# stefantaubert/waveglow

Measured on AMD Instinct MI355X. Metric: audio samples/sec/GPU (22.05 kHz) WaveGlow-256 infer; real-time factor, higher is better.
Workload: dtype f16 MFMA operands, f32 accumulate/flow state, fp16 I/O; 1 GPU; configs[1]: 256ch WaveGlow.infer, batch=16/GPU mels 80x864, fp16 I/O, sigma=0.6; parallelism=utterance-sharded x1, no collective

## Files before the change

### waveglow_amd/csrc/api.cpp

```cpp
#include <cmath>
#include <cstdarg>
#include <cstring>

#include "wg_host.h"

using namespace wg;

namespace {
thread_local std::string g_err;
}

int wg::fail(int code, const char* fmt, ...) {
  char buf[512];
  va_list ap;
  va_start(ap, fmt);
  vsnprintf(buf, sizeof buf, fmt, ap);
  va_end(ap);
  g_err = buf;
  return code;
}

namespace {

bool invert(const std::vector<double>& A, int n, std::vector<double>& inv, double& logabsdet, int& sign) {
// ... 195 lines not shown
  if (c.n_flows < 1 || c.n_early_every < 1 || c.n_early_size < 0 || c.n_early_size % 2 != 0)
    return fail(WG_ERR_INVALID, "bad flow configuration");
  std::vector<int> ck = flow_channels(c);
  if (ck.back() < 2 || ck.back() % 2 != 0) return fail(WG_ERR_INVALID, "flow configuration leaves %d channels", ck.back());
  wg_handle* h = new wg_handle();
  h->cfg = c;
  h->device = device_id;
  {
    int ncu = 0;
    if (hipDeviceGetAttribute(&ncu, hipDeviceAttributeMultiprocessorCount, device_id) == hipSuccess && ncu > 0) h->n_cu = ncu;
  }
  h->NS = c.n_mel_channels * c.n_group;
  h->c_k = ck;
  if (const char* e = getenv("WG_FORCE_BN")) h->force_bn = atoi(e);
  if (const char* e = getenv("WG_NO_START_FOLD")) h->fold_start = !(*e == '1');
  h->expected.push_back("upsample.weight");
  h->expected.push_back("upsample.bias");
  for (int k = 0; k < c.n_flows; ++k) {
    const std::string ks = std::to_string(k);
    h->expected.push_back("convinv." + ks + ".conv.weight");
    const std::string p = "WN." + ks + ".";
    for (const char* n : {"start", "cond_layer", "end"}) {
      h->expected.push_back(p + n + ".weight");
      h->expected.push_back(p + n + ".bias");
    }
    for (int i = 0; i < c.n_layers; ++i) {
      const std::string is = std::to_string(i);
      h->expected.push_back(p + "in_layers." + is + ".weight");
      h->expected.push_back(p + "in_layers." + is + ".bias");
      h->expected.push_back(p + "res_skip_layers." + is + ".weight");
// ... 329 lines not shown
}

size_t wg_infer_workspace_bytes(const wg_handle* h, int32_t B, int32_t n_frames) {
  if (!h || B < 1 || n_frames < 1) return 0;
  const int L = n_frames * h->cfg.upsample_stride / h->cfg.n_group;
  RowGeom g = make_geom(h->cfg, B, L, n_frames);
  return carve(h, g, nullptr).bytes;
}

size_t wg_forward_workspace_bytes(const wg_handle* h, int32_t B, int32_t n_frames, int32_t audio_len) {
  if (!h || B < 1 || n_frames < 1 || audio_len < h->cfg.n_group || audio_len % h->cfg.n_group) return 0;
  RowGeom g = make_geom(h->cfg, B, audio_len / h->cfg.n_group, n_frames);
  return carve(h, g, nullptr).bytes;
}

static int run_wn(wg_handle* h, int k, const RowGeom& g, Workspace& w, _Float16*& cur, _Float16*& oth, hipStream_t s) {
  const wg_config& c = h->cfg;
  const int C = c.n_channels;
  int BN = wn_block_n(C);
  if (BN == 128) {
    const int64_t t128 = (int64_t)kPhases * (g.Rp / 128), ncu = h->n_cu > 0 ? h->n_cu : 1;
    const int64_t r128 = (t128 + ncu - 1) / ncu, r64 = (2 * t128 + ncu - 1) / ncu;
    if (t128 < 4 * ncu && 6 * r64 < 10 * r128) BN = 64;
  }
  if (BN == 128 && h->force_bn == 64) BN = 64;
  if (h->force_bn == 128 && wn_block_n(C) == 128) BN = 128;
  const FlowOffsets& fo = h->flows[k];
  for (int i = 0; i < c.n_layers; ++i) {
    const LayerOffsets& lo = fo.layers[i];
    WnLayerArgs a;
    a.x_in = cur;
// ... 14 lines not shown
    a.out = w.OUT;
    a.g = g;
    a.dil = 1 << i;
    a.n_cond_steps = c.n_mel_channels / 16;
    a.M = c.n_mel_channels;
    a.has_res = i < c.n_layers - 1;
    a.row0 = 0;
    a.tiles_per_phase = g.Rp / BN;
    a.sp = nullptr;
    a.save_t = a.save_s = a.save_a = nullptr;
    a.in0 = a.in1 = nullptr;
    a.out0 = nullptr;
    a.n_tiles = kPhases * a.tiles_per_phase;
    a.stamps = h->dbg_stamps;
    a.n_cu = h->n_cu;
    {
      Prof p(h, s, 2);
      HIP_TRY(launch_wn_layer(a, C, BN, s));
    }
    WG_DBG(s, "wn_layer");
    if (a.has_res) std::swap(cur, oth);
  }
  return WG_OK;
}

int wg_infer(wg_handle* h, const void* mel, const void* z_init, const void* const* z_early, int32_t n_z_early,
             float sigma, void* audio, int32_t B, int32_t n_frames, int32_t io_dtype, void* workspace,
             size_t workspace_bytes, void* stream) {
  return wg_infer_ragged(h, mel, nullptr, z_init, z_early, n_z_early, sigma, audio, B, n_frames, io_dtype, workspace,
                         workspace_bytes, stream);
// ... 57 lines not shown
    FlowArgs f = base_flow_args();
    f.first = 1;
    f.z_extra = z_init;
    f.c_next = h->c_k[k];
    f.h_next = f.c_next / 2;
    f.wstart = (const float*)(h->d_blob + h->flows[k].wstart);
    f.bstart = (const float*)(h->d_blob + h->flows[k].bstart);
    f.out_init = (const float*)(h->d_blob + h->flows[k].out_init);
    f.x = cur;
    f.a0p = w.A0;
    f.skip_x = h->fold_start && wn_res_a0(C);
    Prof p(h, s, 1);
    HIP_TRY(launch_flow(f, s));
  }
  WG_DBG(s, "flow");
  for (int k = c.n_flows - 1; k >= 0; --k) {
    int rc = run_wn(h, k, g, w, cur, oth, s);
    if (rc) return rc;
    FlowArgs f = base_flow_args();
    f.c_in = h->c_k[k];
    f.h_in = f.c_in / 2;
    f.winv = (const float*)(h->d_blob + h->flows[k].winv);
    if (is_early(c, k)) {
      f.z_extra = z_early[ze_idx++];
      f.n_extra = c.n_early_size;
      if (!f.z_extra) return fail(WG_ERR_INVALID, "null early-noise tensor");
    }
    f.c_next = f.c_in + f.n_extra;
    f.last = (k == 0);
    if (f.last) {
      if (f.c_next != c.n_group) return fail(WG_ERR_STATE, "flow bookkeeping error");
      f.audio_out = audio;
    } else {
      f.h_next = h->c_k[k - 1] / 2;
      if (h->c_k[k - 1] != f.c_next) return fail(WG_ERR_STATE, "flow bookkeeping error");
      f.wstart = (const float*)(h->d_blob + h->flows[k - 1].wstart);
      f.bstart = (const float*)(h->d_blob + h->flows[k - 1].bstart);
      f.out_init = (const float*)(h->d_blob + h->flows[k - 1].out_init);
      f.x = cur;
      f.a0p = w.A0;
      f.skip_x = h->fold_start && wn_res_a0(C);
    }
    Prof p(h, s, 1);
    HIP_TRY(launch_flow(f, s));
  }
  WG_DBG(s, "flow");
  return WG_OK;
}

int wg_forward(wg_handle* h, const void* mel, const void* audio, float* z, float* const* log_s, float* log_det_W,
               int32_t B, int32_t n_frames, int32_t audio_len, int32_t io_dtype, void* workspace,
               size_t workspace_bytes, void* stream) {
  if (!h) return fail(WG_ERR_INVALID, "null handle");
  if (!h->finalized) return fail(WG_ERR_STATE, "wg_finalize has not been called");
  if (!mel || !audio || !z || !log_s || !log_det_W || !workspace) return fail(WG_ERR_INVALID, "null buffer");
  if (io_dtype != WG_F32 && io_dtype != WG_F16) return fail(WG_ERR_INVALID, "bad io_dtype");
  const wg_config& c = h->cfg;
// ... 160 lines not shown
```

### waveglow_amd/csrc/kernels.hip

```cpp
#include "wg_common.h"

#include <cstdlib>
#include <type_traits>

namespace wg {

typedef _Float16 half8 __attribute__((ext_vector_type(8)));
typedef _Float16 half4 __attribute__((ext_vector_type(4)));
typedef float f32x16 __attribute__((ext_vector_type(16)));
typedef float f32x4 __attribute__((ext_vector_type(4)));

#define WG_GPTR(p) ((const __attribute__((address_space(1))) void*)(p))
#define WG_LPTR(p) ((__attribute__((address_space(3))) void*)(p))

__device__ __forceinline__ float load_io(const void* p, size_t i, int f16) {
  return f16 ? (float)((const _Float16*)p)[i] : ((const float*)p)[i];
}

__device__ __forceinline__ float gate_act(float u, float v) {
  const float e1 = __builtin_amdgcn_exp2f(__builtin_amdgcn_fmed3f(u, -60.0f, 60.0f));
  const float t = 1.0f + __builtin_amdgcn_exp2f(v);
  return (e1 - 1.0f) * __builtin_amdgcn_rcpf(fmaf(e1, t, t));
}

__device__ __forceinline__ void gate_act3(float u, float v, float& th, float& sg, float& ac) {
  const float e1 = __builtin_amdgcn_exp2f(__builtin_amdgcn_fmed3f(u, -60.0f, 60.0f));
  const float t = 1.0f + __builtin_amdgcn_exp2f(__builtin_amdgcn_fmed3f(v, -60.0f, 60.0f));
  const float r = __builtin_amdgcn_rcpf(fmaf(e1, t, t));
  ac = fmaf(e1, r, -r);
  sg = fmaf(e1, r, r);
  th = ac * t;
}

__device__ __forceinline__ void glds16(const void* sbase, unsigned voff, unsigned lds_addr) {
  unsigned keep;
  asm volatile("s_mov_b32 %0, m0\n\ts_mov_b32 m0, %3\n\ts_nop 2\n\tglobal_load_lds_dwordx4 %1, %2\n\ts_mov_b32 m0, %0"
               : "=&s"(keep) : "v"(voff), "s"(sbase), "s"(lds_addr) : "memory");
}
template <int OFF>
__device__ __forceinline__ void gload16(half8& dst, const void* sbase, unsigned voff) {
  asm volatile("s_nop 4\n\tglobal_load_dwordx4 %0, %1, %2 offset:%3" : "=v"(dst) : "v"(voff), "s"(sbase), "i"(OFF) : "memory");
}

#ifdef WG_STAMPS
#define WG_STAMP(i)                                                                              \
  do {                                                                                           \
    __builtin_amdgcn_sched_barrier(0);                                                           \
    unsigned long long _t;                                                                       \
    asm volatile("s_memtime %0\n\ts_waitcnt lgkmcnt(0)" : "=s"(_t)::"memory");                   \
    if (a.stamps && HAS_RES && tid == 0) a.stamps[(size_t)tile * 8 + (i)] = _t;                        \
    __builtin_amdgcn_sched_barrier(0);                                                           \
  } while (0)
#else
#define WG_STAMP(i) do {} while (0)
#endif

constexpr int kTilesPerWG = 2;


__device__ __forceinline__ void mfma16_acc(f32x4& c, const half8& a, const half8& b) {
  c = __builtin_amdgcn_mfma_f32_16x16x32_f16(a, b, c, 0, 0, 0);
}

template <int C> struct WnCfg {
  static constexpr int NW = (C >= 256) ? 8 : C / 32;
  static constexpr int BN = (C >= 512) ? 64 : 128;
};

template <int N> __device__ __forceinline__ void wait_vm() {
  asm volatile("s_waitcnt vmcnt(%0)" :: "i"(N) : "memory");
  __builtin_amdgcn_sched_barrier(0);
// ... 7 lines not shown
  constexpr int MT = PLAIN ? MB : 2 * MB;
  constexpr int NTHREADS = NW * 64;
  constexpr int NT = BN / 32;
  constexpr int CC = CX;
  constexpr int NKX = NTAPS * CC;
  constexpr int BT_BYTES = BN * 128;
  constexpr int ACT_ROW = 2 * C + 16;
  constexpr int K2 = C / 16;
  constexpr int NG = BN * 8 / NTHREADS;
  constexpr int NAH = MT * 2;
  constexpr bool DEFER = (MB == 1);
  static_assert(BN * 8 % NTHREADS == 0 && MB >= 1 && MB <= 2 && NKX >= 1 && (NTAPS == 1 || NTAPS == 3), "tile geometry");
  constexpr bool Q2L = !M16 && DEFER && !DEEP && (NG + NT - 1) / NT == 1 && NT >= NG + MT;
  static_assert(!M16 || (MODE == 0 && MB == 1 && DEFER && !DEEP && NT >= 2), "16x16x32 variant");
  constexpr bool A0G = MODE == 0 && CX == 1 && NTAPS == 1;
  static_assert(!DEEP || (MODE == 0 && DEFER && HAS_COND && MT <= NT && NG <= NT && ((NKX >= 4 && NKX % 2 == 0) || NKX == 1)), "deep prefetch variant");
  static_assert(MODE == 0 || (TPW == 1 && CX == ((MODE == 2 || MODE == 4) ? 2 : 1) * (C / 64)) || (MODE == 3 && CX == 1), "training variants");

  extern __shared__ __attribute__((aligned(16))) char smem[];
  char* const sB = smem;
  char* const sActs = MODE == 4 ? smem : smem + 2 * BT_BYTES;

  const int tid = threadIdx.x;
  const int wave = __builtin_amdgcn_readfirstlane(tid >> 6);
  int lane = tid & 63, ln = lane & 31, lh = lane >> 5;

  unsigned pvoff[NG];
  int pchunk[NG];
  int swB;
  int l15 = lane & 15, l4 = lane >> 4;
// ... 80 lines not shown
  auto column_of = [&](int rr, int p, int& b, int& t) -> bool {
    int rem = rr - tile_b0 * Fp;
    b = tile_b0;
    if (fp_ge_bn) {
      if (rem >= Fp) { rem -= Fp; ++b; }
    } else {
      const int qd = rem / Fp;
      b += qd;
      rem -= qd * Fp;
    }
    const int fq = rem - a.g.Gf;
    t = fq * 32 + p;
    if (!(b < a.g.B && fq >= 0 && fq < a.g.F && t < a.g.L)) return false;
    return a.g.frames == nullptr || t < 32 * a.g.frames[b];
  };

  int tile, tile_end;
  const int tile_step = gridDim.x >> 3;
  int run_start, run_quarter = 0;
  {
    const int bid = blockIdx.x, ntl = a.n_tiles;
    const int xcd = bid & 7, idx = bid >> 3;
    const int qq = ntl >> 3, r = ntl & 7;
    const int start = xcd < r ? xcd * (qq + 1) : r * (qq + 1) + (xcd - r) * qq;
    tile_end = start + (xcd < r ? qq + 1 : qq);
    tile = start + idx;
    run_start = start;
    if (((tile_end - start) & 3) == 0) run_quarter = (tile_end - start) >> 2;
  }
  auto tile_of = [&](int t) { return run_quarter ? run_start + ((t - run_start) & 3) * run_quarter + ((t - run_start) >> 2) : t; };

  half8 q[4][MT];
  int par = 0;
  if (tile < tile_end) {
    const int t0 = tile_of(tile), p0 = t0 / a.tiles_per_phase;
#pragma unroll
    for (int i = 0; i < NG; ++i) stage_B_piece(p0, t0 - p0 * a.tiles_per_phase, 0, 0, i);
  }
  float* const sBias = (float*)(sActs + BN * ACT_ROW);
  if constexpr (!PLAIN) {
    for (int i = tid; i < 2 * C; i += NTHREADS) sBias[i] = a.bias1[i];
    if constexpr (HAS_RES)
      for (int i = tid; i < C; i += NTHREADS) sBias[2 * C + i] = a.bias2[i];
    uint4* const sW = (uint4*)(sBias + 3 * C);
    for (int i = tid; i < (C / 32) * 64; i += NTHREADS) sW[i] = ((const uint4*)a.wEs)[i];
  }
  __syncthreads();

#pragma unroll
  for (int it = 0; it < TPW; ++it, tile += tile_step) {
    if (tile >= tile_end) break;
    if (it > 0) set_lane_ids();
    const int tile_m = tile_of(tile);
    const int p = tile_m / a.tiles_per_phase;
    const int jt = tile_m - p * a.tiles_per_phase;
    const int rr0 = a.row0 + jt * BN;
    tile_b0 = rr0 / Fp;
    const int r0 = kRowPad + p * Rp + rr0;
    const int next_tile = tile + tile_step;
    wA1c_p = (const char*)a.wA1c + (MODE != 0 ? (size_t)0 : (size_t)p * (2 * a.n_cond_steps) * NW * (NAH * 1024));
// ... 431 lines not shown
    const int l15 = laneo & 15, l4 = laneo >> 4;
    char* const acts_lane16 = sActs + l15 * ACT_ROW + (l4 & 1) * 32 + (l4 >> 1) * 8;
    auto write_acts16 = [&](int c, int blk_, int mh, const half8& o) {
      typedef _Float16 half4_t __attribute__((ext_vector_type(4)));
      const half4_t lo = {o[0], o[1], o[2], o[3]}, hi = {o[4], o[5], o[6], o[7]};
      char* ap = acts_lane16 + c * 32 * ACT_ROW + blk_ * 64 + mh * 16;
      *(half4_t*)(ap) = lo;
      *(half4_t*)(ap + 16 * ACT_ROW) = hi;
    };
    constexpr int NGRP = (BN / 16 + NW - 1) / NW;
    constexpr bool kWesEarly = (C / 32) * 4 <= 32;
    half8 wes[C / 32];
    float4 es_o[NGRP];
    float4* es_op[NGRP];
    bool es_valid[NGRP];
    auto es_prefetch_w = [&](int s_) { wes[s_] = ((const half8*)(sBias + 3 * C) + laneo)[s_ * 64]; };
    auto es_prefetch = [&]() {
#pragma unroll
      for (int gi = 0; gi < NGRP; ++gi) {
        const int grp = wave + gi * NW;
        es_valid[gi] = false;
        es_o[gi] = make_float4(0.f, 0.f, 0.f, 0.f);
        es_op[gi] = nullptr;
        if (grp < BN / 16) {
          int cb, ct;
          es_valid[gi] = column_of(rr0 + grp * 16 + l15, p, cb, ct) && laneo < 32;
          es_op[gi] = (float4*)(a.out + ((size_t)cb * a.g.L + ct) * 8 + 4 * l4);
          if (es_valid[gi]) es_o[gi] = *es_op[gi];
        }
      }
    };
    auto es_compute = [&]() {
#pragma unroll
      for (int s = 0; s < C / 32; ++s) es_prefetch_w(s);
#pragma unroll
      for (int gi = 0; gi < NGRP; ++gi) {
        const int grp = wave + gi * NW;
        if (grp < BN / 16) {
          const char* ep = sActs + (grp * 16 + l15) * ACT_ROW + l4 * 16;
          f32x4 d = {0.f, 0.f, 0.f, 0.f};
#pragma unroll
          for (int s = 0; s < C / 32; ++s) {
            const half8 bfe = *(const half8*)(ep + s * 64);
            d = __builtin_amdgcn_mfma_f32_16x16x32_f16(wes[s], bfe, d, 0, 0, 0);
          }
#pragma unroll
          for (int r = 0; r < 4; ++r) d[r] += __shfl_xor(d[r], 32);
          if (es_valid[gi]) {
            float4 o = es_o[gi];
            o.x += d[0]; o.y += d[1]; o.z += d[2]; o.w += d[3];
            *es_op[gi] = o;
          }
        }
      }
    };
    auto read_acts32 = [&](int nt, int k16) -> half8 {
      return *(const half8*)(acts_rd + nt * 32 * ACT_ROW + k16 * 32);
    };
    constexpr int PF = 8 / MB;
    half8 xres[RES_A0 ? 1 : MB][RES_A0 ? 1 : NT][2];
    half8 a0f[RES_A0 ? NT : 1], wst[RES_A0 ? MB : 1];
    half8 a2[MB][PF];
    const half8* const p2 = (const half8*)a.wA2 + (size_t)wave * MB * K2 * 64 + laneo;
    f32x16 acc2[MB][NT];
    if constexpr (PIPE) {
      constexpr int SL = 16;
      const int blk = wave;
// ... 260 lines not shown
#pragma unroll
        for (int mb = 0; mb < MB; ++mb) {
          const half8 af = a2[mb][k % PF];
          if (k + PF < K2) a2[mb][k % PF] = p2[((size_t)mb * K2 + k + PF) * 64];
#pragma unroll
          for (int nt = 0; nt < NT; ++nt)
            acc2[mb][nt] = __builtin_amdgcn_mfma_f32_32x32x16_f16(af, bq[k & 1][nt], acc2[mb][nt], 0, 0, 0);
        }
      }
    }

    if constexpr (!PIPE) {
      WG_STAMP(4);
      if constexpr (!kWesEarly) es_prefetch();
      es_compute();
    }

    if constexpr (!PIPE) WG_STAMP(5);
    if constexpr (HAS_RES && !PIPE) {
#pragma unroll
      for (int nt = 0; nt < NT; ++nt) {
        int cb, ct;
        if (column_of(rr0 + nt * 32 + lno, p, cb, ct)) {
#pragma unroll
          for (int mb = 0; mb < MB; ++mb) {
            const int blk = wave * MB + mb;
            half8 o0, o1;
#pragma unroll
            for (int r = 0; r < 8; ++r) {
              o0[r] = (_Float16)acc2[mb][nt][r];
// ... 8 lines not shown
      }
    }
    if constexpr (!PIPE) WG_STAMP(6);
    }
    __builtin_amdgcn_sched_barrier(0);
  }
}

template <int C, int BN, bool HAS_RES, int TPW, int CX, int MODE = 0, int NTAPS = 3, bool HAS_COND = true, bool DEEP = false>
static hipError_t launch_wn_tttt(const WnLayerArgs& a, hipStream_t s) {
  constexpr int NW = WnCfg<C>::NW;
  constexpr bool M16 = wn_frag16(C, BN) && MODE == 0 && !DEEP;
  if (M16 != (a.frag16 != 0)) return hipErrorInvalidValue;
  if (MODE == 0 && CX == 1 && NTAPS == 1 && wn_res_a0(C) && HAS_RES && !a.wStA) return hipErrorInvalidValue;
  constexpr int smem = MODE == 4 ? (BN * (2 * C + 16) > 2 * BN * 128 ? BN * (2 * C + 16) : 2 * BN * 128)
                                 : 2 * BN * 128 + (MODE >= 2 ? 0 : BN * (2 * C + 16) + 3 * C * 4 + (C / 32) * 1024);
  static bool attr_done_dev[64] = {};
  int cur_dev = 0;
  if (hipGetDevice(&cur_dev) != hipSuccess || cur_dev < 0 || cur_dev >= 64) cur_dev = 0;
  bool& attr_done = attr_done_dev[cur_dev];
  if (!attr_done) {
    hipError_t e = hipFuncSetAttribute((const void*)wn_layer_kernel<C, NW, BN, HAS_RES, TPW, CX, MODE, NTAPS, HAS_COND, DEEP, M16>,
                                       hipFuncAttributeMaxDynamicSharedMemorySize, smem);
    if (e != hipSuccess) return e;
    attr_done = true;
  }
  const int per_label = ((a.n_tiles + 7) / 8 + TPW - 1) / TPW;
  const int grid = 8 * per_label;
  hipLaunchKernelGGL((wn_layer_kernel<C, NW, BN, HAS_RES, TPW, CX, MODE, NTAPS, HAS_COND, DEEP, M16>), dim3(grid), dim3(NW * 64), smem, s, a);
  return hipGetLastError();
}
// ... 85 lines not shown
  if ((kind != 2 && kind != 3 && kind != 4) || !a.out0 || !a.x_tap || (kind == 3 && (!a.in0 || !a.in1))) return hipErrorInvalidValue;
  if ((kind == 2 || kind == 4) && (a.x_chunks_per_tap != 2 * (C / 64) || a.n_cond_steps != 0)) return hipErrorInvalidValue;
  if (kind == 4 && (!a.wat_prev || !a.gout || !a.t_prev || !a.s_prev || !a.dpre_prev)) return hipErrorInvalidValue;
  if (kind == 3 && !((a.x_chunks_per_tap == 1 && a.n_cond_steps == 0) || (a.x_chunks_per_tap == C / 64 && a.n_cond_steps == 1 && a.sp)))
    return hipErrorInvalidValue;
  switch (C) {
    case 64: return launch_wn_plain_t<64>(a, kind, bn, s);
    case 128: return launch_wn_plain_t<128>(a, kind, bn, s);
    case 256: return launch_wn_plain_t<256>(a, kind, bn, s);
    case 512: return launch_wn_plain_t<512>(a, kind, bn, s);
  }
  return hipErrorInvalidValue;
}

hipError_t launch_wn_layer(const WnLayerArgs& a, int C, int bn, hipStream_t s) {
  switch (C) {
    case 64: return launch_wn_t<64>(a, bn, s);
    case 128: return launch_wn_t<128>(a, bn, s);
    case 256: return launch_wn_t<256>(a, bn, s);
    case 512: return launch_wn_t<512>(a, bn, s);
  }
  return hipErrorInvalidValue;
}

__global__ void __launch_bounds__(256) mel_pack_kernel(const MelPackArgs a) {
  const int rows_per_utt = a.T + 6;
  const size_t n = (size_t)(3 + a.B * rows_per_utt) * a.M;
  for (size_t idx = (size_t)blockIdx.x * 256 + threadIdx.x; idx < n; idx += (size_t)gridDim.x * 256) {
    const int i = (int)(idx % a.M);
    const int row = (int)(idx / a.M) - 3;
// ... 142 lines not shown

template <int FL_ROWS>
__global__ void __launch_bounds__(FL_ROWS) flow_kernel(const FlowArgs a) {
  __shared__ float4 s_a0[FL_ROWS];
  const int L = a.g.L;
  const size_t nrows = (size_t)a.g.B * L;
  const size_t row0 = (size_t)blockIdx.x * FL_ROWS;
  const int tid = threadIdx.x;

  {
    const size_t row = row0 + tid;
    if (row < nrows) {
      const unsigned r32 = (unsigned)row;
      const int b = (int)(r32 / (unsigned)L), t = (int)(r32 - (unsigned)b * (unsigned)L);
      const bool pad_row = a.g.frames != nullptr && t >= 32 * a.g.frames[b];
      float zn[kMaxGroup];
#pragma unroll
      for (int c = 0; c < kMaxGroup; ++c) zn[c] = 0.0f;
      if (a.direction == 0) {
        if (a.first) {
#pragma unroll
          for (int c = 0; c < kMaxGroup; ++c)
            if (c < a.c_next)
              zn[c] = a.sigma * load_io(a.z_extra, ((size_t)b * a.c_next + c) * L + t, a.io_f16);
        } else {
          float z[kMaxGroup], o[kMaxGroup], v[kMaxGroup], y[kMaxGroup];
          const float4* zp = (const float4*)(a.Z + row * 8);
          const float4* op = (const float4*)(a.out + row * 8);
          float4 z0 = zp[0], z1 = zp[1], o0 = op[0], o1 = op[1];
          z[0] = z0.x; z[1] = z0.y; z[2] = z0.z; z[3] = z0.w; z[4] = z1.x; z[5] = z1.y; z[6] = z1.z; z[7] = z1.w;
          o[0] = o0.x; o[1] = o0.y; o[2] = o0.z; o[3] = o0.w; o[4] = o1.x; o[5] = o1.y; o[6] = o1.z; o[7] = o1.w;
          const int h = a.h_in, c = a.c_in;
#pragma unroll
          for (int j = 0; j < kMaxGroup; ++j) {
            float num = z[j], den = 1.0f;
#pragma unroll
            for (int q = 0; q < 4; ++q)
              if (j >= h && j - h == q) { num = z[j] - o[q]; den = expf(o[j]); }
            v[j] = (j < c) ? num / den : 0.0f;
          }
#pragma unroll
          for (int r = 0; r < kMaxGroup; ++r) {
            float s = 0.0f;
#pragma unroll
            for (int cc = 0; cc < kMaxGroup; ++cc)
              if (r < c && cc < c) s = fmaf(a.winv[r * c + cc], v[cc], s);
            y[r] = s;
          }
          const int ne = a.n_extra;
#pragma unroll
          for (int e = 0; e < kMaxGroup; ++e) {
            float val = 0.0f;
            if (e < ne) val = a.sigma * load_io(a.z_extra, ((size_t)b * ne + e) * L + t, a.io_f16);
#pragma unroll
            for (int r = 0; r < kMaxGroup; ++r)
              if (e >= ne && e - ne == r) val = y[r];
            zn[e] = val;
          }
        }
        if (a.last) {
          if (pad_row) {
#pragma unroll
            for (int c = 0; c < 8; ++c) zn[c] = 0.0f;
          }
          if (a.io_f16) {
            half8 o;
#pragma unroll
            for (int c = 0; c < 8; ++c) o[c] = (_Float16)zn[c];
            *(half8*)((_Float16*)a.audio_out + row * 8) = o;
          } else {
            float4* ap = (float4*)((float*)a.audio_out + row * 8);
            ap[0] = make_float4(zn[0], zn[1], zn[2], zn[3]);
            ap[1] = make_float4(zn[4], zn[5], zn[6], zn[7]);
          }
        }
      } else {
        float z[kMaxGroup];
        if (a.first) {
#pragma unroll
          for (int c = 0; c < 8; ++c)
            z[c] = load_io(a.audio_in, (size_t)b * L * 8 + (size_t)t * 8 + c, a.io_f16);
        } else {
          const float4* zp = (const float4*)(a.Z + row * 8);
          const float4* op = (const float4*)(a.out + row * 8);
          float4 z0 = zp[0], z1 = zp[1], o0 = op[0], o1 = op[1];
          float o[kMaxGroup];
          z[0] = z0.x; z[1] = z0.y; z[2] = z0.z; z[3] = z0.w; z[4] = z1.x; z[5] = z1.y; z[6] = z1.z; z[7] = z1.w;
          o[0] = o0.x; o[1] = o0.y; o[2] = o0.z; o[3] = o0.w; o[4] = o1.x; o[5] = o1.y; o[6] = o1.z; o[7] = o1.w;
          const int h = a.h_in;
// ... 22 lines not shown
            for (int q = 0; q < kMaxGroup; ++q)
              if (q - np == e) val = z[q];
            zs[e] = val;
          }
#pragma unroll
          for (int r = 0; r < kMaxGroup; ++r) {
            float s = 0.0f;
#pragma unroll
            for (int cc = 0; cc < kMaxGroup; ++cc)
              if (r < c && cc < c) s = fmaf(a.winv[r * c + cc], zs[cc], s);
            zn[r] = s;
          }
        }
      }
      if (!a.last) {
        float4* zp = (float4*)(a.Z_w + row * 8);
        zp[0] = make_float4(zn[0], zn[1], zn[2], zn[3]);
        zp[1] = make_float4(zn[4], zn[5], zn[6], zn[7]);
        float4* op = (float4*)(a.out_w + row * 8);
        op[0] = make_float4(a.out_init[0], a.out_init[1], a.out_init[2], a.out_init[3]);
        op[1] = make_float4(a.out_init[4], a.out_init[5], a.out_init[6], a.out_init[7]);
        s_a0[tid] = make_float4(zn[0], zn[1], zn[2], zn[3]);
        if (a.a0p && !pad_row) {
          half8 o;
#pragma unroll
          for (int e = 0; e < 8; ++e) o[e] = (_Float16)0.0f;
          const int hn = a.h_next;
          o[0] = (_Float16)zn[0];
          if (hn > 1) o[1] = (_Float16)zn[1];
          if (hn > 2) o[2] = (_Float16)zn[2];
          if (hn > 3) o[3] = (_Float16)zn[3];
          o[4] = (_Float16)1.0f;
          const size_t prow = (size_t)kRowPad + (size_t)(t & 31) * a.g.Rp + (size_t)b * a.g.Fp + a.g.Gf + (t >> 5);
          *(half8*)(a.a0p + prow * 64) = o;
          *(half8*)(a.a0p + prow * 64 + 8) = o;
        }
      }
    }
  }
  if (a.last || a.skip_x) return;
  __syncthreads();
  start_rows<FL_ROWS>(s_a0, row0, nrows, L, a.g, a.wstart, a.bstart, a.C, a.h_next, a.x);
}

template <int FL_ROWS>
__global__ void __launch_bounds__(FL_ROWS) start_replay_kernel(const FlowArgs a) {
  __shared__ float4 s_a0[FL_ROWS];
  const int L = a.g.L;
  const size_t nrows = (size_t)a.g.B * L;
  const size_t row0 = (size_t)blockIdx.x * FL_ROWS;
  const size_t row = row0 + threadIdx.x;
// ... 72 lines not shown
```

### waveglow_amd/csrc/wg_common.h

```cpp
#pragma once
#include <hip/hip_runtime.h>
#include <stdint.h>

namespace wg {

__host__ __device__ inline int pos_to_chan(int P) {
  const int blk = P >> 5, p = P & 31;
  const int h = p >> 4, g = (p >> 2) & 3, i = p & 3;
  return (blk << 5) + 8 * g + 4 * h + i;
}
__host__ __device__ inline int chan_to_pos(int c) {
  const int blk = c >> 5, o = c & 31;
  const int g = o >> 3, h = (o >> 2) & 1, i = o & 3;
  return (blk << 5) + 16 * h + 4 * g + i;
}

constexpr int kMaxGroup = 8;
constexpr int kBK = 64;

struct RowGeom {
  int B;
  int L;
  int F;
  int Gf;
  int Fp;
  int Rp;
  int R;
  int T;
  const int* frames;
};
constexpr int kRowPad = 16;
constexpr int kPhases = 32;

constexpr bool wn_frag16(int C, int BN) { return C == 256 && BN == 128; }

constexpr bool wn_res_a0(int) { return true; }

struct WnLayerArgs {
  const _Float16* x_in;
  const _Float16* x_tap;
  int x_chunks_per_tap;
  _Float16* x_out;
  const _Float16* melT;
  const _Float16* wA1;
  const _Float16* wA1c;
  const float* bias1;
  const _Float16* wA2;
  const float* bias2;
  const _Float16* wEs;
  float* out;
  RowGeom g;
  int dil;
  int n_cond_steps;
  int M;
  int has_res;
  int row0;
  int tiles_per_phase;
  int n_tiles;
  int n_cu;
  int frag16 = 0;
  int a0_fold = 0;
  const _Float16* wStA = nullptr;
  unsigned long long* stamps;
  const _Float16* sp;
  _Float16* save_t;
  _Float16* save_s;
  _Float16* save_a;
  const _Float16* in0;
  const _Float16* in1;
  _Float16* out0;
  const _Float16* wat_prev;
  const _Float16* gout;
  const _Float16* t_prev;
  const _Float16* s_prev;
  _Float16* dpre_prev;
};

// ... 58 lines not shown
```

### waveglow_amd/csrc/wg_host.h

```cpp
#pragma once
#include <hip/hip_runtime.h>

#include <cstdio>
#include <cstdlib>
#include <map>
#include <string>
#include <vector>

#include "../../include/waveglow_amd.h"
#include "wg_common.h"

namespace wg {

int fail(int code, const char* fmt, ...) __attribute__((format(printf, 2, 3)));

#define HIP_TRY(expr)                                                                          \
  do {                                                                                         \
    hipError_t _e = (expr);                                                                    \
    if (_e != hipSuccess) return wg::fail(WG_ERR_HIP, "%s: %s", #expr, hipGetErrorString(_e)); \
  } while (0)

inline bool dbg_sync() {
  static int v = -1;
  if (v < 0) { const char* e = getenv("WG_DEBUG_SYNC"); v = e && *e == '1'; }
// ... 55 lines not shown
  int device;
  int NS;
  std::vector<int> c_k;
  std::vector<std::string> expected;
  std::map<std::string, wg::HostTensor> tensors;
  bool finalized = false;
  char* d_blob = nullptr;
  size_t blob_bytes = 0;
  char* d_cond = nullptr;
  char* d_cond16 = nullptr;
  size_t cond_layer_bytes = 0, cond_flow_bytes = 0;
  std::vector<wg::FlowOffsets> flows;
  int n_cu = 256;
  int force_bn = 0;
  bool fold_start = true;
  unsigned long long* dbg_stamps = nullptr;
  bool prof = false;
  unsigned prof_mask = ~0u;
  std::vector<hipEvent_t> ev;
  std::vector<int> ev_class;
  size_t ev_used = 0;
  double prof_ms[8] = {0, 0, 0, 0, 0, 0, 0, 0};
  int64_t prof_n[8] = {0, 0, 0, 0, 0, 0, 0, 0};
  hipStream_t aux[3] = {nullptr, nullptr, nullptr};
  std::vector<hipEvent_t> sync_ev;
  size_t sync_next = 0;
  hipEvent_t mark_ev[16] = {nullptr, nullptr, nullptr, nullptr, nullptr, nullptr, nullptr, nullptr,
                            nullptr, nullptr, nullptr, nullptr, nullptr, nullptr, nullptr, nullptr};
  static constexpr int kPins = 4;
  void* pin[kPins] = {nullptr, nullptr, nullptr, nullptr};
// ... 16 lines not shown
```

Measured before the change: 78.94 million samples/s.

## Fuse inverse affine-coupling and invertible-conv step into last WN layer epilogue

The last WN layer of each flow (no residual) now performs the flow inverse step in its epilogue. It stages the end-conv output in LDS, applies the coupling inverse and the 1x1 inverse conv per column, and writes the next Z state, the A0 input, or the audio directly. This removes a separate flow kernel launch per flow and a round trip of the OUT buffer through global memory. The costs are extra LDS, an extra barrier, and the args struct in the WN kernel, which could hurt occupancy or add register pressure. The fusion can be disabled with an env var.

```diff
diff --git a/waveglow_amd/csrc/api.cpp b/waveglow_amd/csrc/api.cpp
--- a/waveglow_amd/csrc/api.cpp
+++ b/waveglow_amd/csrc/api.cpp
@@ -233,6 +233,7 @@
   h->c_k = ck;
   if (const char* e = getenv("WG_FORCE_BN")) h->force_bn = atoi(e);
   if (const char* e = getenv("WG_NO_START_FOLD")) h->fold_start = !(*e == '1');
+  if (const char* e = getenv("WG_NO_FLOW_FUSE")) h->fuse_flow = !(*e == '1');
   h->expected.push_back("upsample.weight");
   h->expected.push_back("upsample.bias");
   for (int k = 0; k < c.n_flows; ++k) {
@@ -592,7 +593,8 @@
   return carve(h, g, nullptr).bytes;
 }
 
-static int run_wn(wg_handle* h, int k, const RowGeom& g, Workspace& w, _Float16*& cur, _Float16*& oth, hipStream_t s) {
+static int run_wn(wg_handle* h, int k, const RowGeom& g, Workspace& w, _Float16*& cur, _Float16*& oth, hipStream_t s,
+                  const FlowStepArgs* fuse = nullptr) {
   const wg_config& c = h->cfg;
   const int C = c.n_channels;
   int BN = wn_block_n(C);
@@ -637,6 +639,10 @@
     a.n_tiles = kPhases * a.tiles_per_phase;
     a.stamps = h->dbg_stamps;
     a.n_cu = h->n_cu;
+    if (fuse && !a.has_res) {
+      a.fuse_flow = 1;
+      a.fl = *fuse;
+    }
     {
       Prof p(h, s, 2);
       HIP_TRY(launch_wn_layer(a, C, BN, s));
@@ -724,9 +730,8 @@
     HIP_TRY(launch_flow(f, s));
   }
   WG_DBG(s, "flow");
+  const bool fuse = h->fuse_flow && h->fold_start && wn_res_a0(C) && c.n_layers >= 2;
   for (int k = c.n_flows - 1; k >= 0; --k) {
-    int rc = run_wn(h, k, g, w, cur, oth, s);
-    if (rc) return rc;
     FlowArgs f = base_flow_args();
     f.c_in = h->c_k[k];
     f.h_in = f.c_in / 2;
@@ -747,10 +752,17 @@
       f.wstart = (const float*)(h->d_blob + h->flows[k - 1].wstart);
       f.bstart = (const float*)(h->d_blob + h->flows[k - 1].bstart);
       f.out_init = (const float*)(h->d_blob + h->flows[k - 1].out_init);
-      f.x = cur;
       f.a0p = w.A0;
       f.skip_x = h->fold_start && wn_res_a0(C);
     }
+    FlowStepArgs fs;
+    fs.Z = f.Z; fs.Z_w = f.Z_w; fs.out_w = f.out_w; fs.winv = f.winv; fs.z_extra = f.z_extra; fs.n_extra = f.n_extra;
+    fs.sigma = f.sigma; fs.c_in = f.c_in; fs.h_in = f.h_in; fs.h_next = f.h_next; fs.out_init = f.out_init; fs.a0p = f.a0p;
+    fs.audio_out = f.audio_out; fs.io_f16 = f.io_f16; fs.last = f.last;
+    int rc = run_wn(h, k, g, w, cur, oth, s, fuse ? &fs : nullptr);
+    if (rc) return rc;
+    if (fuse) continue;
+    f.x = cur;
     Prof p(h, s, 1);
     HIP_TRY(launch_flow(f, s));
   }
diff --git a/waveglow_amd/csrc/kernels.hip b/waveglow_amd/csrc/kernels.hip
--- a/waveglow_amd/csrc/kernels.hip
+++ b/waveglow_amd/csrc/kernels.hip
@@ -1,5 +1,6 @@
 #include "wg_common.h"
 
+#include <cstddef>
 #include <cstdlib>
 #include <type_traits>
 
@@ -12,6 +13,9 @@
 
 #define WG_GPTR(p) ((const __attribute__((address_space(1))) void*)(p))
 #define WG_LPTR(p) ((__attribute__((address_space(3))) void*)(p))
+typedef __attribute__((address_space(3))) f32x4 lds_f32x4;
+typedef __attribute__((address_space(3))) unsigned lds_u32;
+typedef const float* __attribute__((address_space(3))) lds_cfptr;
 
 __device__ __forceinline__ float load_io(const void* p, size_t i, int f16) {
   return f16 ? (float)((const _Float16*)p)[i] : ((const float*)p)[i];
@@ -40,6 +44,94 @@
 template <int OFF>
 __device__ __forceinline__ void gload16(half8& dst, const void* sbase, unsigned voff) {
   asm volatile("s_nop 4\n\tglobal_load_dwordx4 %0, %1, %2 offset:%3" : "=v"(dst) : "v"(voff), "s"(sbase), "i"(OFF) : "memory");
+}
+
+__device__ __forceinline__ void flow_store_audio(void* audio_out, int io_f16, size_t row, const float (&zn)[kMaxGroup]) {
+  if (io_f16) {
+    half8 o;
+#pragma unroll
+    for (int c = 0; c < 8; ++c) o[c] = (_Float16)zn[c];
+    *(half8*)((_Float16*)audio_out + row * 8) = o;
+  } else {
+    float4* ap = (float4*)((float*)audio_out + row * 8);
+    ap[0] = make_float4(zn[0], zn[1], zn[2], zn[3]);
+    ap[1] = make_float4(zn[4], zn[5], zn[6], zn[7]);
+  }
+}
+__device__ __forceinline__ void flow_store_state(float* Z_w, float* out_w, const float* out_init, _Float16* a0p, int h_next,
+                                                 size_t row, size_t prow, bool plane_ok, const float (&zn)[kMaxGroup]) {
+  float4* zp = (float4*)(Z_w + row * 8);
+  zp[0] = make_float4(zn[0], zn[1], zn[2], zn[3]);
+  zp[1] = make_float4(zn[4], zn[5], zn[6], zn[7]);
+  float4* op = (float4*)(out_w + row * 8);
+  op[0] = make_float4(out_init[0], out_init[1], out_init[2], out_init[3]);
+  op[1] = make_float4(out_init[4], out_init[5], out_init[6], out_init[7]);
+  if (a0p && plane_ok) {
+    half8 o;
+#pragma unroll
+    for (int e = 0; e < 8; ++e) o[e] = (_Float16)0.0f;
+    o[0] = (_Float16)zn[0];
+    if (h_next > 1) o[1] = (_Float16)zn[1];
+    if (h_next > 2) o[2] = (_Float16)zn[2];
+    if (h_next > 3) o[3] = (_Float16)zn[3];
+    o[4] = (_Float16)1.0f;
+    *(half8*)(a0p + prow * 64) = o;
+    *(half8*)(a0p + prow * 64 + 8) = o;
+  }
+}
+template <int CIN>
+__device__ __forceinline__ void flow_inverse_row_c(const FlowStepArgs& f, const float* winv, const float* out_init,
+                                                   const float4 z0, const float4 z1, const float4 o0, const float4 o1, size_t row,
+                                                   int b, int t, int L, bool pad_row, size_t prow, float (&zn)[kMaxGroup]) {
+  float z[kMaxGroup], o[kMaxGroup], v[kMaxGroup], y[kMaxGroup];
+  z[0] = z0.x; z[1] = z0.y; z[2] = z0.z; z[3] = z0.w; z[4] = z1.x; z[5] = z1.y; z[6] = z1.z; z[7] = z1.w;
+  o[0] = o0.x; o[1] = o0.y; o[2] = o0.z; o[3] = o0.w; o[4] = o1.x; o[5] = o1.y; o[6] = o1.z; o[7] = o1.w;
+  const int h = CIN ? CIN / 2 : f.h_in, c = CIN ? CIN : f.c_in;
+#pragma unroll
+  for (int j = 0; j < kMaxGroup; ++j) {
+    float num = z[j], den = 1.0f;
+#pragma unroll
+    for (int q = 0; q < 4; ++q)
+      if (j >= h && j - h == q) { num = z[j] - o[q]; den = expf(o[j]); }
+    v[j] = (j < c) ? num / den : 0.0f;
+  }
+#pragma unroll
+  for (int r = 0; r < kMaxGroup; ++r) {
+    float s = 0.0f;
+#pragma unroll
+    for (int cc = 0; cc < kMaxGroup; ++cc)
+      if (r < c && cc < c) s = fmaf(winv[r * c + cc], v[cc], s);
+    y[r] = s;
+  }
+  const int ne = f.n_extra;
+#pragma unroll
+  for (int e = 0; e < kMaxGroup; ++e) {
+    float val = 0.0f;
+    if (e < ne) val = f.sigma * load_io(f.z_extra, ((size_t)b * ne + e) * L + t, f.io_f16);
+#pragma unroll
+    for (int r = 0; r < kMaxGroup; ++r)
+      if (e >= ne && e - ne == r) val = y[r];
+    zn[e] = val;
+  }
+  if (f.last) {
+    if (pad_row) {
+#pragma unroll
+      for (int e = 0; e < 8; ++e) zn[e] = 0.0f;
+    }
+    flow_store_audio(f.audio_out, f.io_f16, row, zn);
+  } else {
+    flow_store_state(f.Z_w, f.out_w, out_init, f.a0p, f.h_next, row, prow, !pad_row, zn);
+  }
+}
+__device__ __forceinline__ void flow_inverse_row(const FlowStepArgs& f, const float* winv, const float* out_init,
+                                                 const float4 z0, const float4 z1, const float4 o0, const float4 o1, size_t row,
+                                                 int b, int t, int L, bool pad_row, size_t prow, float (&zn)[kMaxGroup]) {
+  switch (f.h_in * 2 == f.c_in ? f.c_in : 0) {
+    case 8: flow_inverse_row_c<8>(f, winv, out_init, z0, z1, o0, o1, row, b, t, L, pad_row, prow, zn); break;
+    case 6: flow_inverse_row_c<6>(f, winv, out_init, z0, z1, o0, o1, row, b, t, L, pad_row, prow, zn); break;
+    case 4: flow_inverse_row_c<4>(f, winv, out_init, z0, z1, o0, o1, row, b, t, L, pad_row, prow, zn); break;
+    default: flow_inverse_row_c<0>(f, winv, out_init, z0, z1, o0, o1, row, b, t, L, pad_row, prow, zn); break;
+  }
 }
 
 #ifdef WG_STAMPS
@@ -55,6 +147,9 @@
 #define WG_STAMP(i) do {} while (0)
 #endif
 
+constexpr int kFlowLdsArgs = 64 + 8;
+constexpr int kFlowArgWords = (sizeof(FlowStepArgs) + 3) / 4;
+constexpr int kFlowLds = kFlowLdsArgs + (kFlowArgWords + 3) / 4 * 4;
 constexpr int kTilesPerWG = 2;
 
 
@@ -92,6 +187,8 @@
   constexpr bool Q2L = !M16 && DEFER && !DEEP && (NG + NT - 1) / NT == 1 && NT >= NG + MT;
   static_assert(!M16 || (MODE == 0 && MB == 1 && DEFER && !DEEP && NT >= 2), "16x16x32 variant");
   constexpr bool A0G = MODE == 0 && CX == 1 && NTAPS == 1;
+  constexpr bool FUSE = MODE == 0 && !HAS_RES;
+  static_assert(NTHREADS >= kFlowLdsArgs && (!FUSE || NTHREADS >= BN), "one thread per staged float / per column of the fused flow step");
   static_assert(!DEEP || (MODE == 0 && DEFER && HAS_COND && MT <= NT && NG <= NT && ((NKX >= 4 && NKX % 2 == 0) || NKX == 1)), "deep prefetch variant");
   static_assert(MODE == 0 || (TPW == 1 && CX == ((MODE == 2 || MODE == 4) ? 2 : 1) * (C / 64)) || (MODE == 3 && CX == 1), "training variants");
 
@@ -202,6 +299,11 @@
     if (!(b < a.g.B && fq >= 0 && fq < a.g.F && t < a.g.L)) return false;
     return a.g.frames == nullptr || t < 32 * a.g.frames[b];
   };
+  auto column_kind = [&](int rr, int p, int& b, int& t) -> int {
+    if (column_of(rr, p, b, t)) return 2;
+    const int fq = (t - p) >> 5;
+    return (b < a.g.B && fq >= 0 && fq < a.g.F && t < a.g.L) ? 1 : 0;
+  };
 
   int tile, tile_end;
   const int tile_step = gridDim.x >> 3;
@@ -226,12 +328,22 @@
     for (int i = 0; i < NG; ++i) stage_B_piece(p0, t0 - p0 * a.tiles_per_phase, 0, 0, i);
   }
   float* const sBias = (float*)(sActs + BN * ACT_ROW);
+  float* const sFlow = sBias + 3 * C + (C / 32) * 256;
   if constexpr (!PLAIN) {
     for (int i = tid; i < 2 * C; i += NTHREADS) sBias[i] = a.bias1[i];
     if constexpr (HAS_RES)
       for (int i = tid; i < C; i += NTHREADS) sBias[2 * C + i] = a.bias2[i];
     uint4* const sW = (uint4*)(sBias + 3 * C);
     for (int i = tid; i < (C / 32) * 64; i += NTHREADS) sW[i] = ((const uint4*)a.wEs)[i];
+    if constexpr (FUSE) {
+      if (a.fuse_flow && tid < kFlowLdsArgs) {
+        float v = 0.0f;
+        if (tid < 64) { if (tid < a.fl.c_in * a.fl.c_in) v = a.fl.winv[tid]; }
+        else if (!a.fl.last) v = a.fl.out_init[tid - 64];
+        sFlow[tid] = v;
+      }
+      if (a.fuse_flow && tid == 0) *(FlowStepArgs*)(sFlow + kFlowLdsArgs) = a.fl;
+    }
   }
   __syncthreads();
 
@@ -693,6 +805,8 @@
     float4 es_o[NGRP];
     float4* es_op[NGRP];
     bool es_valid[NGRP];
+    int fl_kind = 0, fl_b = 0, fl_t = 0;
+    float4 fl_z0 = make_float4(0.f, 0.f, 0.f, 0.f), fl_z1 = fl_z0;
     auto es_prefetch_w = [&](int s_) { wes[s_] = ((const half8*)(sBias + 3 * C) + laneo)[s_ * 64]; };
     auto es_prefetch = [&]() {
 #pragma unroll
@@ -708,6 +822,17 @@
           if (es_valid[gi]) es_o[gi] = *es_op[gi];
         }
       }
+      if constexpr (FUSE) {
+        if (a.fuse_flow && wave * 64 < BN) {
+          fl_kind = column_kind(rr0 + wave * 64 + laneo, p, fl_b, fl_t);
+          if (fl_kind == 2) {
+            const float* const Zp = *(const lds_cfptr*)WG_LPTR(sFlow + kFlowLdsArgs + offsetof(FlowStepArgs, Z) / 4);
+            const float4* zp = (const float4*)(Zp + ((size_t)fl_b * a.g.L + fl_t) * 8);
+            fl_z0 = zp[0];
+            fl_z1 = zp[1];
+          }
+        }
+      }
     };
     auto es_compute = [&]() {
 #pragma unroll
@@ -725,11 +850,53 @@
           }
 #pragma unroll
           for (int r = 0; r < 4; ++r) d[r] += __shfl_xor(d[r], 32);
-          if (es_valid[gi]) {
+          bool to_lds = false;
+          if constexpr (FUSE) to_lds = a.fuse_flow != 0;
+          if (to_lds) {
+            if (laneo < 32) {
+              float4 o = es_o[gi];
+              o.x += d[0]; o.y += d[1]; o.z += d[2]; o.w += d[3];
+              *(lds_f32x4*)WG_LPTR(sActs + (grp * 16 + l15) * ACT_ROW + l4 * 16) = f32x4{o.x, o.y, o.z, o.w};
+            }
+          } else if (es_valid[gi]) {
             float4 o = es_o[gi];
             o.x += d[0]; o.y += d[1]; o.z += d[2]; o.w += d[3];
             *es_op[gi] = o;
           }
+        }
+      }
+    };
+    auto flow_args = [&]() -> FlowStepArgs {
+      unsigned w[kFlowArgWords];
+#pragma unroll
+      for (int i = 0; i < kFlowArgWords; ++i) w[i] = ((const lds_u32*)WG_LPTR(sFlow + kFlowLdsArgs))[i];
+      FlowStepArgs f;
+      __builtin_memcpy(&f, w, sizeof f);
+      f.n_extra = __builtin_amdgcn_readfirstlane(f.n_extra);
+      f.c_in = __builtin_amdgcn_readfirstlane(f.c_in);
+      f.h_in = __builtin_amdgcn_readfirstlane(f.h_in);
+      f.h_next = __builtin_amdgcn_readfirstlane(f.h_next);
+      f.io_f16 = __builtin_amdgcn_readfirstlane(f.io_f16);
+      f.last = __builtin_amdgcn_readfirstlane(f.last);
+      return f;
+    };
+    auto flow_tail = [&]() {
+      asm volatile("s_waitcnt lgkmcnt(0)" ::: "memory");
+      __builtin_amdgcn_s_barrier();
+      asm volatile("" ::: "memory");
+      if (wave * 64 < BN && fl_kind != 0) {
+        const FlowStepArgs f = flow_args();
+        const size_t row = (size_t)fl_b * a.g.L + fl_t;
+        if (fl_kind == 2) {
+          const lds_f32x4* op = (const lds_f32x4*)WG_LPTR(sActs + (wave * 64 + laneo) * ACT_ROW);
+          const f32x4 q0 = op[0], q1 = op[1];
+          float zn[kMaxGroup];
+          flow_inverse_row(f, sFlow, sFlow + 64, fl_z0, fl_z1, make_float4(q0[0], q0[1], q0[2], q0[3]),
+                           make_float4(q1[0], q1[1], q1[2], q1[3]), row, fl_b, fl_t, a.g.L, false,
+                           (size_t)r0 + wave * 64 + laneo, zn);
+        } else if (f.last) {
+          const float zero[kMaxGroup] = {0.f, 0.f, 0.f, 0.f, 0.f, 0.f, 0.f, 0.f};
+          flow_store_audio(f.audio_out, f.io_f16, row, zero);
         }
       }
     };
@@ -1020,6 +1187,7 @@
       WG_STAMP(4);
       if constexpr (!kWesEarly) es_prefetch();
       es_compute();
+      if constexpr (FUSE) if (a.fuse_flow) flow_tail();
     }
 
     if constexpr (!PIPE) WG_STAMP(5);
@@ -1058,7 +1226,7 @@
   if (M16 != (a.frag16 != 0)) return hipErrorInvalidValue;
   if (MODE == 0 && CX == 1 && NTAPS == 1 && wn_res_a0(C) && HAS_RES && !a.wStA) return hipErrorInvalidValue;
   constexpr int smem = MODE == 4 ? (BN * (2 * C + 16) > 2 * BN * 128 ? BN * (2 * C + 16) : 2 * BN * 128)
-                                 : 2 * BN * 128 + (MODE >= 2 ? 0 : BN * (2 * C + 16) + 3 * C * 4 + (C / 32) * 1024);
+                                 : 2 * BN * 128 + (MODE >= 2 ? 0 : BN * (2 * C + 16) + 3 * C * 4 + (C / 32) * 1024 + kFlowLds * 4);
   static bool attr_done_dev[64] = {};
   int cur_dev = 0;
   if (hipGetDevice(&cur_dev) != hipSuccess || cur_dev < 0 || cur_dev >= 64) cur_dev = 0;
@@ -1174,6 +1342,13 @@
 }
 
 hipError_t launch_wn_layer(const WnLayerArgs& a, int C, int bn, hipStream_t s) {
+  if (a.fuse_flow) {
+    const FlowStepArgs& f = a.fl;
+    if (a.has_res || a.a0_fold) return hipErrorInvalidValue;
+    if (!f.Z || f.Z_w != f.Z || f.out_w != a.out || !f.winv || f.c_in < 2 || f.c_in > kMaxGroup || f.h_in * 2 != f.c_in) return hipErrorInvalidValue;
+    if (f.n_extra < 0 || f.c_in + f.n_extra > kMaxGroup || (f.n_extra && !f.z_extra)) return hipErrorInvalidValue;
+    if (f.last ? !f.audio_out : (!f.out_init || f.h_next < 1 || f.h_next > 4)) return hipErrorInvalidValue;
+  }
   switch (C) {
     case 64: return launch_wn_t<64>(a, bn, s);
     case 128: return launch_wn_t<128>(a, bn, s);
@@ -1346,6 +1521,8 @@
       const unsigned r32 = (unsigned)row;
       const int b = (int)(r32 / (unsigned)L), t = (int)(r32 - (unsigned)b * (unsigned)L);
       const bool pad_row = a.g.frames != nullptr && t >= 32 * a.g.frames[b];
+      const size_t prow = (size_t)kRowPad + (size_t)(t & 31) * a.g.Rp + (size_t)b * a.g.Fp + a.g.Gf + (t >> 5);
+      bool stored = false;
       float zn[kMaxGroup];
 #pragma unroll
       for (int c = 0; c < kMaxGroup; ++c) zn[c] = 0.0f;
@@ -1356,55 +1533,22 @@
             if (c < a.c_next)
               zn[c] = a.sigma * load_io(a.z_extra, ((size_t)b * a.c_next + c) * L + t, a.io_f16);
         } else {
-          float z[kMaxGroup], o[kMaxGroup], v[kMaxGroup], y[kMaxGroup];
+          FlowStepArgs f;
+          f.Z = a.Z; f.Z_w = a.Z_w; f.out_w = a.out_w; f.winv = a.winv; f.z_extra = a.z_extra; f.n_extra = a.n_extra;
+          f.sigma = a.sigma; f.c_in = a.c_in; f.h_in = a.h_in; f.h_next = a.h_next; f.out_init = a.out_init; f.a0p = a.a0p;
+          f.audio_out = a.audio_out; f.io_f16 = a.io_f16; f.last = a.last;
           const float4* zp = (const float4*)(a.Z + row * 8);
           const float4* op = (const float4*)(a.out + row * 8);
-          float4 z0 = zp[0], z1 = zp[1], o0 = op[0], o1 = op[1];
-          z[0] = z0.x; z[1] = z0.y; z[2] = z0.z; z[3] = z0.w; z[4] = z1.x; z[5] = z1.y; z[6] = z1.z; z[7] = z1.w;
-          o[0] = o0.x; o[1] = o0.y; o[2] = o0.z; o[3] = o0.w; o[4] = o1.x; o[5] = o1.y; o[6] = o1.z; o[7] = o1.w;
-          const int h = a.h_in, c = a.c_in;
-#pragma unroll
-          for (int j = 0; j < kMaxGroup; ++j) {
-            float num = z[j], den = 1.0f;
-#pragma unroll
-            for (int q = 0; q < 4; ++q)
-              if (j >= h && j - h == q) { num = z[j] - o[q]; den = expf(o[j]); }
-            v[j] = (j < c) ? num / den : 0.0f;
-          }
-#pragma unroll
-          for (int r = 0; r < kMaxGroup; ++r) {
-            float s = 0.0f;
-#pragma unroll
-            for (int cc = 0; cc < kMaxGroup; ++cc)
-              if (r < c && cc < c) s = fmaf(a.winv[r * c + cc], v[cc], s);
-            y[r] = s;
-          }
-          const int ne = a.n_extra;
-#pragma unroll
-          for (int e = 0; e < kMaxGroup; ++e) {
-            float val = 0.0f;
-            if (e < ne) val = a.sigma * load_io(a.z_extra, ((size_t)b * ne + e) * L + t, a.io_f16);
-#pragma unroll
-            for (int r = 0; r < kMaxGroup; ++r)
-              if (e >= ne && e - ne == r) val = y[r];
-            zn[e] = val;
-          }
-        }
-        if (a.last) {
+          const float4 z0 = zp[0], z1 = zp[1], o0 = op[0], o1 = op[1];
+          flow_inverse_row(f, a.winv, a.out_init, z0, z1, o0, o1, row, b, t, L, pad_row, prow, zn);
+          stored = true;
+        }
+        if (a.last && !stored) {
           if (pad_row) {
 #pragma unroll
             for (int c = 0; c < 8; ++c) zn[c] = 0.0f;
           }
-          if (a.io_f16) {
-            half8 o;
-#pragma unroll
-            for (int c = 0; c < 8; ++c) o[c] = (_Float16)zn[c];
-            *(half8*)((_Float16*)a.audio_out + row * 8) = o;
-          } else {
-            float4* ap = (float4*)((float*)a.audio_out + row * 8);
-            ap[0] = make_float4(zn[0], zn[1], zn[2], zn[3]);
-            ap[1] = make_float4(zn[4], zn[5], zn[6], zn[7]);
-          }
+          flow_store_audio(a.audio_out, a.io_f16, row, zn);
         }
       } else {
         float z[kMaxGroup];
@@ -1457,27 +1601,8 @@
         }
       }
       if (!a.last) {
-        float4* zp = (float4*)(a.Z_w + row * 8);
-        zp[0] = make_float4(zn[0], zn[1], zn[2], zn[3]);
-        zp[1] = make_float4(zn[4], zn[5], zn[6], zn[7]);
-        float4* op = (float4*)(a.out_w + row * 8);
-        op[0] = make_float4(a.out_init[0], a.out_init[1], a.out_init[2], a.out_init[3]);
-        op[1] = make_float4(a.out_init[4], a.out_init[5], a.out_init[6], a.out_init[7]);
+        if (!stored) flow_store_state(a.Z_w, a.out_w, a.out_init, a.a0p, a.h_next, row, prow, !pad_row, zn);
         s_a0[tid] = make_float4(zn[0], zn[1], zn[2], zn[3]);
-        if (a.a0p && !pad_row) {
-          half8 o;
-#pragma unroll
-          for (int e = 0; e < 8; ++e) o[e] = (_Float16)0.0f;
-          const int hn = a.h_next;
-          o[0] = (_Float16)zn[0];
-          if (hn > 1) o[1] = (_Float16)zn[1];
-          if (hn > 2) o[2] = (_Float16)zn[2];
-          if (hn > 3) o[3] = (_Float16)zn[3];
-          o[4] = (_Float16)1.0f;
-          const size_t prow = (size_t)kRowPad + (size_t)(t & 31) * a.g.Rp + (size_t)b * a.g.Fp + a.g.Gf + (t >> 5);
-          *(half8*)(a.a0p + prow * 64) = o;
-          *(half8*)(a.a0p + prow * 64 + 8) = o;
-        }
       }
     }
   }
diff --git a/waveglow_amd/csrc/wg_common.h b/waveglow_amd/csrc/wg_common.h
--- a/waveglow_amd/csrc/wg_common.h
+++ b/waveglow_amd/csrc/wg_common.h
@@ -36,6 +36,23 @@
 
 constexpr bool wn_res_a0(int) { return true; }
 
+struct FlowStepArgs {
+  const float* Z;
+  float* Z_w;
+  float* out_w;
+  const float* winv;
+  const void* z_extra;
+  int n_extra;
+  float sigma;
+  int c_in, h_in;
+  int h_next;
+  const float* out_init;
+  _Float16* a0p;
+  void* audio_out;
+  int io_f16;
+  int last;
+};
+
 struct WnLayerArgs {
   const _Float16* x_in;
   const _Float16* x_tap;
@@ -61,6 +78,8 @@
   int frag16 = 0;
   int a0_fold = 0;
   const _Float16* wStA = nullptr;
+  int fuse_flow = 0;
+  FlowStepArgs fl = {};
   unsigned long long* stamps;
   const _Float16* sp;
   _Float16* save_t;
diff --git a/waveglow_amd/csrc/wg_host.h b/waveglow_amd/csrc/wg_host.h
--- a/waveglow_amd/csrc/wg_host.h
+++ b/waveglow_amd/csrc/wg_host.h
@@ -93,6 +93,7 @@
   int n_cu = 256;
   int force_bn = 0;
   bool fold_start = true;
+  bool fuse_flow = true;
   unsigned long long* dbg_stamps = nullptr;
   bool prof = false;
   unsigned prof_mask = ~0u;
```

Result: no change. 78.78 million samples/s (-0.2%).
